# OxfordML/GPz

Measured on AMD Instinct MI355X. Metric: objective+gradient evals/sec, higher is better.
Workload: dtype f64

## Files before the change

gpz_amd/csrc/k_moments_ring.hip:

```cpp
#include "gpz_dev.h"
#include "gpz_kernels.h"

#define RG_ROWS 8
#define RG_SLOTS 4
#define RG_JB 2
#define RG_COLS 32
#define RG_SLOT_DOUBLES 640
#define RG_SIDE 512
#define RG_SIDE_RS 96
#define RG_GROUP_REQ 5
#define RG_LDS_BYTES 81920
#define RG_GLDS(g, l) __builtin_amdgcn_global_load_lds((const __attribute__((address_space(1))) void *)(g), (__attribute__((address_space(3))) void *)(l), 16, 0, 0)
static_assert(RG_LDS_BYTES == 4 * RG_SLOTS * RG_SLOT_DOUBLES * 8 && RG_COLS == 16 * RG_JB && RG_SIDE == 2 * RG_ROWS * RG_COLS, "ring size");

template <int D>
__global__ __launch_bounds__(256, 2) void k_moments_ring(RingMomentArgs a) {
    constexpr int NF = 1 + D + D * (D + 1) / 2, XL = D + 2;
    constexpr int NFB = NF >= 64 ? NF / 16 : (NF + 15) / 16;
    constexpr int NL = NF > 16 * NFB ? NF - 16 * NFB : 0;
    static_assert(RG_ROWS * XL <= RG_SIDE_RS, "side block");
    extern __shared__ double rg_smem[];
    const int tid = threadIdx.x, lane = tid & 63, wave = __builtin_amdgcn_readfirstlane(tid >> 6), li = lane & 15, lk = lane >> 4;
    const int ncg = (a.m + 4 * RG_COLS - 1) / (4 * RG_COLS);
    const int cg = blockIdx.x % ncg, chunk = blockIdx.x / ncg;
    const int j0 = cg * (4 * RG_COLS) + wave * RG_COLS;
    if (j0 >= a.m) return;
    double *const ring = rg_smem + wave * (RG_SLOTS * RG_SLOT_DOUBLES);
    const int r_begin = chunk * a.rows_per_chunk;
    const int r_end = min(a.n, r_begin + a.rows_per_chunk);
    const int ng = (r_end - r_begin + RG_ROWS - 1) / RG_ROWS;
    double wj[RG_JB], vj[RG_JB];
#pragma unroll
    for (int cb = 0; cb < RG_JB; ++cb) {
        const int j = min(j0 + 16 * cb + li, a.m - 1);
        wj[cb] = a.w[j];
        vj[cb] = a.v ? a.v[j] : 0.0;
    }
    int fia[NFB], fib[NFB];
#pragma unroll
    for (int fb = 0; fb < NFB; ++fb) {
        const int f = 16 * fb + li;
        int ia = 0, ib = 0;
        if (f >= NF) ia = ib = XL - 1;
        else if (f >= 1) {
            if (f <= D) ia = f;
            else {
                int e2 = f - 1 - D, aa = 0;
                while (e2 >= D - aa) { e2 -= D - aa; ++aa; }
                ia = aa + 1; ib = aa + e2 + 1;
            }
        }
        fia[fb] = ia; fib[fb] = ib;
    }
    int lia[NL > 0 ? NL : 1], lib[NL > 0 ? NL : 1];
#pragma unroll
    for (int t = 0; t < NL; ++t) {
        int e2 = 16 * NFB + t - 1 - D, aa = 0;
        while (e2 >= D - aa) { e2 -= D - aa; ++aa; }
        lia[t] = aa + 1; lib[t] = aa + e2 + 1;
    }
    d4_t acc[RG_JB][NFB];
    double ev[RG_JB][NL + 2];
#pragma unroll
    for (int cb = 0; cb < RG_JB; ++cb) {
#pragma unroll
        for (int fb = 0; fb < NFB; ++fb) acc[cb][fb] = d4_t{0.0, 0.0, 0.0, 0.0};
#pragma unroll
        for (int t = 0; t < NL + 2; ++t) ev[cb][t] = 0.0;
    }
    const unsigned colj = (unsigned)min(j0 + 2 * (lane & 15), a.ld - 2);
    const unsigned voff = (unsigned)(lane >> 4) * (unsigned)a.ld + colj;
    const bool is_rs = lane >= 48;
    const unsigned soff = is_rs ? 2u * (unsigned)(lane - 48) : min(2u * (unsigned)lane, (unsigned)(RG_ROWS * XL - 2));
    const double *const sbase = is_rs ? a.rowscal : a.Xs;
    const unsigned srow = is_rs ? 4u : (unsigned)XL;
    const long last = (long)r_end - 1;
    auto stage_half = [&](int g, int slot, int h) {
        const long rg = (long)r_begin + (long)g * RG_ROWS + 4 * h;
        double *const l0 = ring + slot * RG_SLOT_DOUBLES + 4 * h * RG_COLS;
        if (rg + 4 <= (long)r_end) {
            const size_t ro = (size_t)rg * (size_t)a.ld;
            RG_GLDS(a.Phi + ro + voff, l0);
            RG_GLDS(a.T + ro + voff, l0 + RG_ROWS * RG_COLS);
        } else {
            long row = rg + (lane >> 4);
            row = row < last ? row : last;
            const size_t ro = (size_t)row * (size_t)a.ld + colj;
            RG_GLDS(a.Phi + ro, l0);
            RG_GLDS(a.T + ro, l0 + RG_ROWS * RG_COLS);
        }
    };
    auto stage_side = [&](int g, int slot) {
        const long rg = (long)r_begin + (long)g * RG_ROWS;
        double *const l0 = ring + slot * RG_SLOT_DOUBLES + RG_SIDE;
        long e = rg * (long)srow + (long)soff;
        const long elast = (long)r_end * (long)srow - 2;
        e = e < elast ? e : elast;
        RG_GLDS(sbase + e, l0);
    };
    auto kstep = [&](const double *s0, int kk, int rows_left) {
        const int rr = 4 * kk + lk;
        const bool valid = rr < rows_left;
        const double *xr = s0 + RG_SIDE + rr * XL;
        const double *rs = s0 + RG_SIDE + RG_SIDE_RS + rr * 4;
        const double r0 = rs[0], r1 = rs[1], r2 = rs[2];
        const double ob = valid ? r0 : 0.0, cc = valid ? r1 : 0.0, db = valid ? r2 : 0.0;
        double fr[NFB], fl[NL > 0 ? NL : 1];
#pragma unroll
        for (int fb = 0; fb < NFB; ++fb) fr[fb] = xr[fia[fb]] * xr[fib[fb]];
#pragma unroll
        for (int t = 0; t < NL; ++t) fl[t] = xr[lia[t]] * xr[lib[t]];
        const double *pp = s0 + rr * RG_COLS + li;
        double phn = pp[0], ttn = pp[RG_ROWS * RG_COLS];
        __builtin_amdgcn_sched_barrier(0);
#pragma unroll
        for (int cb = 0; cb < RG_JB; ++cb) {
            const double ph = phn, tt = ttn;
            if (cb + 1 < RG_JB) { phn = pp[16 * (cb + 1)]; ttn = pp[RG_ROWS * RG_COLS + 16 * (cb + 1)]; }
            const double dp = fma(-ob, tt, fma(db, vj[cb], -cc * wj[cb])) * ph;
#pragma unroll
            for (int fb = 0; fb < NFB; ++fb) acc[cb][fb] = MFMA_F64(dp, fr[fb], acc[cb][fb]);
#pragma unroll
            for (int t = 0; t < NL; ++t) ev[cb][t] = fma(dp, fl[t], ev[cb][t]);
            ev[cb][NL] = fma(ph, cc, ev[cb][NL]);
            ev[cb][NL + 1] = fma(ph, db, ev[cb][NL + 1]);
            __builtin_amdgcn_sched_barrier(0);
        }
    };
    for (int g = 0; g < RG_SLOTS; ++g)
        if (g < ng) { stage_half(g, g, 0); stage_half(g, g, 1); stage_side(g, g); }
    for (int g = 0; g < ng; ++g) {
        const int ahead = ng - 1 - g;
        if (ahead >= 3) asm volatile("s_waitcnt vmcnt(15)" ::: "memory");
        else if (ahead == 2) asm volatile("s_waitcnt vmcnt(10)" ::: "memory");
        else if (ahead == 1) asm volatile("s_waitcnt vmcnt(5)" ::: "memory");
        else asm volatile("s_waitcnt vmcnt(0)" ::: "memory");
        const int slot = g % RG_SLOTS;
        const double *s0 = ring + slot * RG_SLOT_DOUBLES;
        const int rows_left = r_end - r_begin - g * RG_ROWS;
        const bool more = g + RG_SLOTS < ng;
        kstep(s0, 0, rows_left);
        asm volatile("s_waitcnt lgkmcnt(0)" ::: "memory");
        if (more) stage_half(g + RG_SLOTS, slot, 0);
        kstep(s0, 1, rows_left);
        asm volatile("s_waitcnt lgkmcnt(0)" ::: "memory");
        if (more) { stage_half(g + RG_SLOTS, slot, 1); stage_side(g + RG_SLOTS, slot); }
    }
    double *rec = a.slab + (size_t)chunk * a.m * (NF + 2);
#pragma unroll
    for (int cb = 0; cb < RG_JB; ++cb) {
#pragma unroll
        for (int r = 0; r < 4; ++r) {
            const int j = j0 + 16 * cb + lk + 4 * r;
            if (j < a.m) {
                double *o = rec + (size_t)j * (NF + 2);
#pragma unroll
                for (int fb = 0; fb < NFB; ++fb)
                    if (16 * fb + li < NF) o[16 * fb + li] = acc[cb][fb][r];
            }
        }
        const int j = j0 + 16 * cb + li;
#pragma unroll
        for (int t = 0; t < NL + 2; ++t) {
            double s = ev[cb][t];
            s += __shfl_xor(s, 16, 64);
            s += __shfl_xor(s, 32, 64);
            if (lk == 0 && j < a.m) rec[(size_t)j * (NF + 2) + (NF - NL) + t] = s;
        }
    }
}

__global__ __launch_bounds__(1024) void k_ring_finish(const double *__restrict__ slab, int nrec, int m, int d, int nf, const double *__restrict__ P,
                                                      const double *__restrict__ xmu, int nm, int mp, double *__restrict__ mom,
                                                      double *__restrict__ cols, int accumulate) {
    __shared__ double part[32][72];
    __shared__ double R[72];
    const int tid = threadIdx.x, j = blockIdx.x, nv = nf + 2;
    const int L = 1024 / nv < 32 ? 1024 / nv : 32;
    const int f = tid % nv, sl = tid / nv;
    if (sl < L) {
        const double *p = slab + (size_t)j * nv + f;
        const size_t stride = (size_t)m * nv;
        double s0 = 0.0, s1 = 0.0, s2 = 0.0, s3 = 0.0;
        int r = sl;
        for (; r + 3 * L < nrec; r += 4 * L) {
            s0 += p[(size_t)r * stride];
            s1 += p[(size_t)(r + L) * stride];
            s2 += p[(size_t)(r + 2 * L) * stride];
            s3 += p[(size_t)(r + 3 * L) * stride];
        }
        for (; r < nrec; r += L) s0 += p[(size_t)r * stride];
        part[sl][f] = (s0 + s1) + (s2 + s3);
    }
    __syncthreads();
    if (tid < nv) {
        double t = 0.0;
        for (int q = 0; q < L; ++q) t += part[q][tid];
        R[tid] = t;
    }
    __syncthreads();
    const int q = tid;
    if (q >= nm + 2) return;
    if (q >= nm) {
        cols[(size_t)(q - nm) * mp + j] = R[nf + (q - nm)];
        return;
    }
    double val;
    if (q < d) {
        const double qc = P[(size_t)j * d + q] - xmu[q];
        val = R[1 + q] - qc * R[0];
    } else {
        int e = q - d, aa = 0;
        while (e >= d - aa) { e -= d - aa; ++aa; }
        const int bb = aa + e;
        const double qa = P[(size_t)j * d + aa] - xmu[aa], qb = P[(size_t)j * d + bb] - xmu[bb];
        val = R[1 + q] - qa * R[1 + bb] - qb * R[1 + aa] + qa * qb * R[0];
    }
    mom[(size_t)j * nm + q] = accumulate ? mom[(size_t)j * nm + q] + val : val;
}

bool moments_ring_fits(int kind, int de, int mp) { return kind == GPZ_KIND_COV && (de == 8 || de == 10) && mp > 256; }
int moments_ring_cols() { return 4 * RG_COLS; }
int moments_ring_features(int de) { return 1 + de + de * (de + 1) / 2; }

template <int D>
static int ring_launch(hipStream_t st, const RingMomentArgs &a, dim3 g) {
    if (hipFuncSetAttribute((const void *)k_moments_ring<D>, hipFuncAttributeMaxDynamicSharedMemorySize, RG_LDS_BYTES) != hipSuccess) return -1;
    hipLaunchKernelGGL(k_moments_ring<D>, g, dim3(256), RG_LDS_BYTES, st, a);
    return hipGetLastError() == hipSuccess ? 0 : -1;
}

int launch_moments_ring(hipStream_t st, const RingMomentArgs &a) {
    if (a.nchunk <= 0) return 0;
    dim3 g((unsigned)((a.m + 4 * RG_COLS - 1) / (4 * RG_COLS)) * (unsigned)a.nchunk);
    switch (a.d) {
        case 8: return ring_launch<8>(st, a, g);
        case 10: return ring_launch<10>(st, a, g);
        default: return -1;
    }
}

void launch_ring_finish(hipStream_t st, const double *slab, int nrec, int m, int d, const double *P, const double *xmu, int nm, int mp,
                        double *mom, double *cols, int accumulate) {
    hipLaunchKernelGGL(k_ring_finish, dim3(m), dim3(1024), 0, st, slab, nrec, m, d, moments_ring_features(d), P, xmu, nm, mp, mom, cols, accumulate);
}
```

Baseline: 18.65.

## Unroll ring loop by slot count with precomputed LDS addresses and split tail

Rewrites the main ring-buffer loop so each pass unrolls over the four slots, letting slot offsets be compile-time constants. LDS addresses for phi, side data and feature gathers are precomputed once as 32-bit address-space-3 pointers, and global source pointers advance incrementally instead of being recomputed. Full row groups take a specialized path without row-bound checks, and the final partial group runs after the loop. The goal is to cut per-iteration address arithmetic, branching and modulo work in the hot loop, at the cost of larger code, more register pressure and more complex tail handling.

```diff
diff --git a/gpz_amd/csrc/k_moments_ring.hip b/gpz_amd/csrc/k_moments_ring.hip
--- a/gpz_amd/csrc/k_moments_ring.hip
+++ b/gpz_amd/csrc/k_moments_ring.hip
@@ -11,6 +11,8 @@
 #define RG_GROUP_REQ 5
 #define RG_LDS_BYTES 81920
 #define RG_GLDS(g, l) __builtin_amdgcn_global_load_lds((const __attribute__((address_space(1))) void *)(g), (__attribute__((address_space(3))) void *)(l), 16, 0, 0)
+typedef const __attribute__((address_space(3))) double *lds_cd;
+#define RG_LDS(x) ((lds_cd)(__UINTPTR_TYPE__)(x))
 static_assert(RG_LDS_BYTES == 4 * RG_SLOTS * RG_SLOT_DOUBLES * 8 && RG_COLS == 16 * RG_JB && RG_SIDE == 2 * RG_ROWS * RG_COLS, "ring size");
 
 template <int D>
@@ -129,22 +131,112 @@
     };
     for (int g = 0; g < RG_SLOTS; ++g)
         if (g < ng) { stage_half(g, g, 0); stage_half(g, g, 1); stage_side(g, g); }
-    for (int g = 0; g < ng; ++g) {
-        const int ahead = ng - 1 - g;
-        if (ahead >= 3) asm volatile("s_waitcnt vmcnt(15)" ::: "memory");
-        else if (ahead == 2) asm volatile("s_waitcnt vmcnt(10)" ::: "memory");
-        else if (ahead == 1) asm volatile("s_waitcnt vmcnt(5)" ::: "memory");
-        else asm volatile("s_waitcnt vmcnt(0)" ::: "memory");
-        const int slot = g % RG_SLOTS;
-        const double *s0 = ring + slot * RG_SLOT_DOUBLES;
-        const int rows_left = r_end - r_begin - g * RG_ROWS;
-        const bool more = g + RG_SLOTS < ng;
-        kstep(s0, 0, rows_left);
+    const int nw = (r_end - r_begin) / RG_ROWS, nrem = r_end - r_begin - nw * RG_ROWS;
+    const unsigned ringb = (unsigned)(__UINTPTR_TYPE__)(__attribute__((address_space(3))) double *)ring;
+    unsigned pb = ringb + 8u * (unsigned)(lk * RG_COLS + li);
+    unsigned xb = ringb + 8u * (unsigned)(RG_SIDE + lk * XL);
+    unsigned rb = ringb + 8u * (unsigned)(RG_SIDE + RG_SIDE_RS + lk * 4);
+    unsigned fa[NFB], fo[NFB];
+#pragma unroll
+    for (int fb = 0; fb < NFB; ++fb) { fa[fb] = xb + 8u * (unsigned)fia[fb]; fo[fb] = xb + 8u * (unsigned)fib[fb]; }
+    asm volatile("" : "+v"(pb), "+v"(xb), "+v"(rb));
+#pragma unroll
+    for (int fb = 0; fb < NFB; ++fb) asm volatile("" : "+v"(fa[fb]), "+v"(fo[fb]));
+    auto kstep_whole = [&](int so, int kk) {
+        const lds_cd rs = RG_LDS(rb) + (so + 16 * kk);
+        const lds_cd xr = RG_LDS(xb) + (so + 4 * kk * XL);
+        double xa[NFB], xo[NFB], la[NL > 0 ? NL : 1], lo[NL > 0 ? NL : 1];
+#pragma unroll
+        for (int fb = 0; fb < NFB; ++fb) { xa[fb] = (RG_LDS(fa[fb]))[so + 4 * kk * XL]; xo[fb] = (RG_LDS(fo[fb]))[so + 4 * kk * XL]; }
+#pragma unroll
+        for (int t = 0; t < NL; ++t) { la[t] = xr[lia[t]]; lo[t] = xr[lib[t]]; }
+        const double ob = rs[0], cc = rs[1], db = rs[2];
+        const lds_cd pp = RG_LDS(pb) + (so + 4 * kk * RG_COLS);
+        double phn = pp[0], ttn = pp[RG_ROWS * RG_COLS];
+        __builtin_amdgcn_sched_barrier(0);
+        double fr[NFB], fl[NL > 0 ? NL : 1];
+#pragma unroll
+        for (int fb = 0; fb < NFB; ++fb) fr[fb] = xa[fb] * xo[fb];
+#pragma unroll
+        for (int t = 0; t < NL; ++t) fl[t] = la[t] * lo[t];
+        __builtin_amdgcn_sched_barrier(0);
+#pragma unroll
+        for (int cb = 0; cb < RG_JB; ++cb) {
+            const double ph = phn, tt = ttn;
+            if (cb + 1 < RG_JB) { phn = pp[16 * (cb + 1)]; ttn = pp[RG_ROWS * RG_COLS + 16 * (cb + 1)]; }
+            const double dp = fma(-ob, tt, fma(db, vj[cb], -cc * wj[cb])) * ph;
+#pragma unroll
+            for (int fb = 0; fb < NFB; ++fb) acc[cb][fb] = MFMA_F64(dp, fr[fb], acc[cb][fb]);
+#pragma unroll
+            for (int t = 0; t < NL; ++t) ev[cb][t] = fma(dp, fl[t], ev[cb][t]);
+            ev[cb][NL] = fma(ph, cc, ev[cb][NL]);
+            ev[cb][NL + 1] = fma(ph, db, ev[cb][NL + 1]);
+            __builtin_amdgcn_sched_barrier(0);
+        }
+    };
+    const unsigned vo = 8u * voff;
+    const int rcl0 = max(min(lk, nrem - 1), 0), rcl1 = max(min(4 + lk, nrem - 1), 0);
+    const unsigned to0 = 8u * ((unsigned)rcl0 * (unsigned)a.ld + colj), to1 = 8u * ((unsigned)rcl1 * (unsigned)a.ld + colj);
+    const size_t gstep = (size_t)RG_ROWS * (size_t)a.ld * 8;
+    const char *gphi = reinterpret_cast<const char *>(a.Phi) + ((size_t)r_begin / RG_ROWS + RG_SLOTS) * gstep + ((size_t)r_begin % RG_ROWS) * (gstep / RG_ROWS);
+    const char *gt = reinterpret_cast<const char *>(a.T) + (gphi - reinterpret_cast<const char *>(a.Phi));
+    const unsigned sstep = 8u * RG_ROWS * srow;
+    const char *sp = reinterpret_cast<const char *>(sbase + ((long)r_begin + RG_SLOTS * RG_ROWS) * (long)srow + (long)soff);
+    const char *spt;
+    {
+        long e = ((long)r_begin + (long)nw * RG_ROWS) * (long)srow + (long)soff;
+        const long elast = (long)r_end * (long)srow - 2;
+        e = e < elast ? e : elast;
+        spt = reinterpret_cast<const char *>(sbase + e);
+    }
+    auto pass = [&](int g, bool steady) {
+#pragma unroll
+        for (int s = 0; s < RG_SLOTS; ++s) {
+            const int gq = g + s + RG_SLOTS;
+            const bool whole = steady || gq < nw, part = !steady && gq == nw && nrem > 0;
+            double *const l0 = ring + s * RG_SLOT_DOUBLES;
+            if (steady || g + s < nw) {
+                const int ahead = ng - 1 - (g + s);
+                if (steady || ahead >= 3) asm volatile("s_waitcnt vmcnt(15)" ::: "memory");
+                else if (ahead == 2) asm volatile("s_waitcnt vmcnt(10)" ::: "memory");
+                else if (ahead == 1) asm volatile("s_waitcnt vmcnt(5)" ::: "memory");
+                else asm volatile("s_waitcnt vmcnt(0)" ::: "memory");
+                kstep_whole(s * RG_SLOT_DOUBLES, 0);
+                asm volatile("s_waitcnt lgkmcnt(0)" ::: "memory");
+                if (whole || part) {
+                    unsigned o = whole ? vo : to0;
+                    asm volatile("" : "+v"(o));
+                    RG_GLDS(gphi + o, l0);
+                    RG_GLDS(gt + o, l0 + RG_ROWS * RG_COLS);
+                }
+                kstep_whole(s * RG_SLOT_DOUBLES, 1);
+                asm volatile("s_waitcnt lgkmcnt(0)" ::: "memory");
+                if (whole) {
+                    unsigned o = vo;
+                    asm volatile("" : "+v"(o));
+                    RG_GLDS(gphi + gstep / 2 + o, l0 + 4 * RG_COLS);
+                    RG_GLDS(gt + gstep / 2 + o, l0 + 4 * RG_COLS + RG_ROWS * RG_COLS);
+                    RG_GLDS(sp, l0 + RG_SIDE);
+                } else if (part) {
+                    unsigned o = to1;
+                    asm volatile("" : "+v"(o));
+                    RG_GLDS(gphi + o, l0 + 4 * RG_COLS);
+                    RG_GLDS(gt + o, l0 + 4 * RG_COLS + RG_ROWS * RG_COLS);
+                    RG_GLDS(spt, l0 + RG_SIDE);
+                }
+                gphi += gstep; gt += gstep; sp += sstep;
+            }
+        }
+    };
+    int g = 0;
+    for (; g + 2 * RG_SLOTS <= nw; g += RG_SLOTS) pass(g, true);
+    for (; g < nw; g += RG_SLOTS) pass(g, false);
+    if (nrem > 0) {
+        asm volatile("s_waitcnt vmcnt(0)" ::: "memory");
+        const double *s0 = ring + (nw % RG_SLOTS) * RG_SLOT_DOUBLES;
+        kstep(s0, 0, nrem);
         asm volatile("s_waitcnt lgkmcnt(0)" ::: "memory");
-        if (more) stage_half(g + RG_SLOTS, slot, 0);
-        kstep(s0, 1, rows_left);
-        asm volatile("s_waitcnt lgkmcnt(0)" ::: "memory");
-        if (more) { stage_half(g + RG_SLOTS, slot, 1); stage_side(g + RG_SLOTS, slot); }
+        kstep(s0, 1, nrem);
     }
     double *rec = a.slab + (size_t)chunk * a.m * (NF + 2);
 #pragma unroll
```

Result: no change. 18.76 (median of 6 runs) (+0.6%).
